# goodgodgd/xpt-mde-2021

Hardware: AMD Instinct MI355X
Metric: train images/sec (5-frame 128x416 snippets) (higher is better)
Workload: dtype bf16; 1 GPU; DepthNet(NASNetMobile)+PoseNetImproved train step, KITTI-raw-shaped 5x128x416 snippets, batch 8/GPU, mono L1+SSIM+smoothness, 4 scales; global_batch=8, per_gpu_batch=8, mode=graph, parallelism=dp1, ranks=1

## Files before the change

### include/xpt_hip.h

```cpp
#ifndef XPT_HIP_H_
#define XPT_HIP_H_

#include <stddef.h>
#include <stdint.h>

#ifdef __cplusplus
extern "C" {
#endif

#define XPT_OK 0
#define XPT_ERR_NULL (-1)
#define XPT_ERR_SHAPE (-2)
#define XPT_ERR_ARG (-3)
#define XPT_ERR_WORKSPACE (-4)
#define XPT_ERR_LAUNCH (-5)

#define XPT_PHOTO_L1 0
#define XPT_PHOTO_L2 1
#define XPT_PHOTO_SSIM 2

int xpt_abi_version(void);
const char* xpt_build_arch(void);

int xpt_pose_rvec2matr_fwd(const float* pose, float* T, int M, void* stream);
// ... 125 lines not shown
int xpt_pwconv_tune(int ksplit_min_cin, int ksplit_max_tiles);
int xpt_pwconv_bn_fwd(const void* x, const void* w, const float* gamma, const float* beta, const float* mean,
                      const float* var, float eps, const void* residual, void* ypre, void* y, long long M, int cin,
                      int cout, long long pitch_x, void* stream);

typedef struct xpt_conv_pack_job {
  const float* src;
  void* fwd;
  void* bwd;
  long long sn, sc, sh, sw;
  int N, T, KW, C, Cp, Np;
  long long first_block;
} xpt_conv_pack_job;
int xpt_conv_pack_job_bytes(void);
int xpt_conv_pack_weights(const void* jobs, int njobs, long long nblocks, void* stream);
int xpt_conv2d_tune(int plan);
int xpt_conv2d_fwd(const void* x, const void* w, const float* bias, void* y, int B, int PH, int PW, int C,
                   long long xpitch, int N, int KH, int KW, int stride, int pad_t, int pad_l, int OH, int OW,
                   long long ypitch, int upsample, float slope, void* stream);
int xpt_conv2d_bwd_data(const void* g, const void* wb, void* dx, int B, int OH, int OW, int Np, long long gpitch,
                        int C, int KH, int KW, int stride, int pad_t, int pad_l, int IH, int IW, long long dxpitch,
                        int fold2x2, void* stream);
int xpt_conv2d_splitk_tune(int enable, int force_split, int min_k, int max_pixels);
size_t xpt_conv2d_splitk_workspace_floats(long long pixels, int out_channels, int red_channels, int taps, int stride);
int xpt_conv2d_fwd_splitk(const void* x, const void* w, const float* bias, void* y, int B, int PH, int PW, int C,
                          long long xpitch, int N, int KH, int KW, int pad_t, int pad_l, int OH, int OW, long long ypitch,
                          int upsample, float slope, float* workspace, size_t workspace_floats, void* stream);
int xpt_conv2d_bwd_data_splitk(const void* g, const void* wb, void* dx, int B, int OH, int OW, int Np, long long gpitch,
                               int C, int KH, int KW, int pad_t, int pad_l, int IH, int IW, long long dxpitch, int fold2x2,
                               float* workspace, size_t workspace_floats, void* stream);
int xpt_conv2d_stream_tune(int enable, int min_tiles, int wgs_per_cu, int max_lds_kib);
int xpt_conv2d_stream_serves(int B, int OH, int OW, int out_channels, int red_channels, int KH, int KW, int stride,
                             int upsample_or_fold);
int xpt_conv2d_fwd_stream(const void* x, const void* w, const float* bias, void* y, int B, int PH, int PW, int C,
                          long long xpitch, int N, int pad_t, int pad_l, int OH, int OW, long long ypitch, int upsample,
                          float slope, void* stream);
int xpt_conv2d_fwd_stream_k5s2(const void* x, const void* w, const float* bias, void* y, int B, int PH, int PW, int C,
                               long long xpitch, int N, int pad_t, int pad_l, int OH, int OW, long long ypitch, float slope,
                               void* stream);
int xpt_conv2d_bwd_data_stream(const void* g, const void* wb, void* dx, int B, int OH, int OW, int Np, long long gpitch, int C,
                               int pad_t, int pad_l, int IH, int IW, long long dxpitch, int fold2x2, void* stream);
int xpt_conv2d_bwd_weight_tune(int max_partial_mib, int target_blocks);
int xpt_conv2d_bwd_weight_splits(int B, int C, int N, int KH, int KW, int stride, int OH, int OW);
int xpt_conv2d_bwd_weight_partials(const void* g, const void* x, float* partials, size_t partial_floats, int B, int PH,
                                   int PW, int C, int Cr, long long xpitch, int N, long long gpitch, int KH, int KW,
                                   int stride, int pad_t, int pad_l, int OH, int OW, int upsample, void* stream);
int xpt_restack_bf16(const float* image5d, void* out, int B, int S, int H, int W, int Cp, void* stream);

int xpt_headconv_tune(int passes, int max_blocks);
int xpt_headconv_bwd_blocks(int B, int H, int W, int C);
int xpt_headconv_fwd(const void* x, long long xpitch, const float* w, const float* bias, float* pre, int B, int H, int W,
                     int C, void* stream);
int xpt_headconv_bwd(const void* x, long long xpitch, const float* w, const float* g, void* dx, float* partials,
// ... 173 lines not shown
```

### xpt_mde_2021_amd/csrc/xpt_conv_splitk.hip

```cpp
#include "xpt_common.h"

namespace {

typedef float f32x16 __attribute__((ext_vector_type(16)));
typedef xpt_h16x8 bf16x8;
typedef unsigned int u32x4 __attribute__((ext_vector_type(4)));

__device__ inline unsigned short f2bf_sk(float f) { return xpt_f2h(f); }

struct SkArgs {
  const unsigned short* x;
  const unsigned short* w;
  float* part;
  long long xpitch;
  long long xbytes, wbytes;
  long long M;
  int B, PH, PW;
  int Hlim, Wlim, shift;
  int C, N, KH, KW;
  int sgn, off_h, off_w;
  int OH, OW, quad;
  int npieces, per_split, nsplit;
  int tiles_m, tiles_n;
};

template <int RN, int NW>
__global__ __launch_bounds__(64 * NW) void conv_splitk_kernel(SkArgs a) {
  constexpr int TN = 64 * RN, TP = 128, PITCH = 64 * 2 + 16;
  constexpr int RPP = 8 * NW, APASS = TN / RPP, BPASS = TP / RPP;
  constexpr int WI = NW == 4 ? RN : 1;
  static_assert(NW == 4 || (NW == 8 && RN == 2), "8 waves: the 128-channel tile only");
  __shared__ __attribute__((aligned(16))) unsigned char lds[(TN + TP) * PITCH];
  unsigned char* const lA = lds;
  unsigned char* const lB = lds + TN * PITCH;
  const int tid = threadIdx.x, lane = tid & 63, wave = tid >> 6;
  const int r = lane & 31, h = lane >> 5;
  const int wm = NW == 4 ? wave >> 1 : wave >> 2, wn = NW == 4 ? wave & 1 : wave & 3;

  const unsigned bid = blockIdx.x;
  int split, tile;
  if (a.nsplit >= 8) {
    split = (int)(bid % (unsigned)a.nsplit);
    tile = (int)(bid / (unsigned)a.nsplit);
  } else {
    const int per = 8 / a.nsplit;
    split = (int)(bid & 7u) % a.nsplit;
    tile = (int)(bid >> 3) * per + (int)(bid & 7u) / a.nsplit;
  }
  if (tile >= a.tiles_m * a.tiles_n) return;
  const int tn = tile % a.tiles_n, tm = tile / a.tiles_n;
  const long long m0 = (long long)tm * TP;
// ... 27 lines not shown

  const int sp = tid & 7, srow = tid >> 3;
  int sb[BPASS], base_h[BPASS], base_w[BPASS];
  bool sok[BPASS];
#pragma unroll
  for (int i = 0; i < BPASS; ++i) {
    int b, oh, ow;
    sok[i] = decode(m0 + srow + RPP * i, b, oh, ow);
    sb[i] = b;
    base_h[i] = oh + a.off_h;
    base_w[i] = ow + a.off_w;
  }
  const int T = a.KH * a.KW;
  constexpr unsigned OOB = 0x40000000u;
  unsigned wro[APASS];
#pragma unroll
  for (int i = 0; i < APASS; ++i) {
    const int n = n0 + srow + RPP * i;
    wro[i] = n < a.N ? (unsigned)n * (unsigned)(T * a.C) * 2u : OOB;
  }
  const __amdgpu_buffer_rsrc_t rx = __builtin_amdgcn_make_buffer_rsrc((void*)a.x, 0, (int)a.xbytes, 0x00020000);
  const __amdgpu_buffer_rsrc_t rw = __builtin_amdgcn_make_buffer_rsrc((void*)a.w, 0, (int)a.wbytes, 0x00020000);

  f32x16 acc[WI][2];
#pragma unroll
  for (int i = 0; i < WI; ++i)
#pragma unroll
    for (int j = 0; j < 2; ++j)
#pragma unroll
      for (int q = 0; q < 16; ++q) acc[i][j][q] = 0.f;

  int pc = p_begin + sp;
  int it, c0;
  {
    const int pcl = pc < a.npieces ? pc : a.npieces - 1;
    it = (int)(((float)pcl + 0.5f) * inv_cp8);
    c0 = (pcl - it * cp8) * 8;
  }
  unsigned xo[BPASS];
  auto set_tap = [&]() {
    const int kh = (int)(((float)it + 0.5f) * inv_kw);
    const int kw = it - kh * a.KW;
#pragma unroll
    for (int i = 0; i < BPASS; ++i) {
      const int th = base_h[i] + a.sgn * kh, tw = base_w[i] + a.sgn * kw;
      const bool ok = sok[i] && th >= 0 && th < a.Hlim && tw >= 0 && tw < a.Wlim;
      const int row = th >> a.shift, col = tw >> a.shift;
      xo[i] = ok ? (unsigned)((sb[i] * a.PH + row) * a.PW + col) * (unsigned)(a.xpitch * 2) : OOB;
    }
  };
  set_tap();
// ... 5 lines not shown
    const unsigned dead = pc < p_end ? 0u : OOB;
    const unsigned cb = (unsigned)(it * a.C + c0) * 2u + dead, xb = (unsigned)c0 * 2u + dead;
#pragma unroll
    for (int i = 0; i < APASS; ++i) st.ra[i] = __builtin_amdgcn_raw_buffer_load_b128(rw, wro[i] + cb, 0, 0);
#pragma unroll
    for (int i = 0; i < BPASS; ++i) st.rb[i] = __builtin_amdgcn_raw_buffer_load_b128(rx, xo[i] + xb, 0, 0);
    pc += 8;
    c0 += 64;
    if (c0 >= a.C) {
      do {
        c0 -= a.C;
        ++it;
      } while (c0 >= a.C);
      it = it < T ? it : T - 1;
      set_tap();
    }
  };
  auto stash = [&](const Stage& st) {
#pragma unroll
    for (int i = 0; i < APASS; ++i) *(u32x4*)(lA + (srow + RPP * i) * PITCH + sp * 16) = st.ra[i];
#pragma unroll
    for (int i = 0; i < BPASS; ++i) *(u32x4*)(lB + (srow + RPP * i) * PITCH + sp * 16) = st.rb[i];
  };
  const unsigned char* const fB = lB + (wm * 64 + r) * PITCH + h * 16;
  const unsigned char* const fA = lA + (wn * 32 * WI + r) * PITCH + h * 16;
  auto multiply = [&]() {
    u32x4 fb[4][2], fa[4][WI];
#pragma unroll
    for (int k16 = 0; k16 < 4; ++k16) {
#pragma unroll
      for (int j = 0; j < 2; ++j) fb[k16][j] = *(const u32x4*)(fB + 32 * j * PITCH + k16 * 32);
#pragma unroll
      for (int i = 0; i < WI; ++i) fa[k16][i] = *(const u32x4*)(fA + 32 * i * PITCH + k16 * 32);
    }
#pragma unroll
    for (int k16 = 0; k16 < 4; ++k16)
#pragma unroll
      for (int i = 0; i < WI; ++i)
#pragma unroll
        for (int j = 0; j < 2; ++j)
          acc[i][j] = XPT_MFMA_32X32X16(__builtin_bit_cast(bf16x8, fa[k16][i]), __builtin_bit_cast(bf16x8, fb[k16][j]),
                                                              acc[i][j]);
  };

  Stage s0, s1;
  if (nchunks > 0) {
    fetch(s0);
    if (nchunks > 1) fetch(s1);
    stash(s0);
    if (nchunks > 2) fetch(s0);
    __syncthreads();
  }
  for (int ck = 0; ck < nchunks; ck += 2) {
    multiply();
    if (ck + 1 < nchunks) {
      __syncthreads();
      stash(s1);
      if (ck + 3 < nchunks) fetch(s1);
      __syncthreads();
      multiply();
      if (ck + 2 < nchunks) {
        __syncthreads();
        stash(s0);
        if (ck + 4 < nchunks) fetch(s0);
        __syncthreads();
      }
    }
  }

  float* const out = a.part + (long long)split * a.M * a.N;
  const bool vec_ok = (a.N & 3) == 0;
#pragma unroll
  for (int j = 0; j < 2; ++j) {
    const long long m = m0 + 64 * wm + 32 * j + r;
    if (m >= a.M) continue;
#pragma unroll
    for (int i = 0; i < WI; ++i) {
#pragma unroll
      for (int qg = 0; qg < 4; ++qg) {
        const int n = n0 + 32 * WI * wn + 32 * i + 8 * qg + 4 * h;
        if (n >= a.N) continue;
        float* dst = out + m * a.N + n;
        if (vec_ok) {
          *(float4*)dst = make_float4(acc[i][j][4 * qg], acc[i][j][4 * qg + 1], acc[i][j][4 * qg + 2], acc[i][j][4 * qg + 3]);
        } else {
#pragma unroll
          for (int e = 0; e < 4; ++e)
            if (n + e < a.N) dst[e] = acc[i][j][4 * qg + e];
        }
      }
    }
  }
}

template <int NS>
__global__ __launch_bounds__(256) void conv_splitk_finish_kernel(const float* __restrict__ part, const float* __restrict__ bias,
                                                                 unsigned short* __restrict__ y, long long ypitch, unsigned Mout,
                                                                 long long M, int N, int quad, float slope) {
  const unsigned n4 = (unsigned)(N + 3) >> 2;
  const unsigned idx = blockIdx.x * 256u + threadIdx.x;
  if (idx >= Mout * n4) return;
  unsigned rem;
  const unsigned mo = xpt_divmod(idx, n4, rem);
  const int n = (int)rem * 4;
  const int nchild = quad ? 4 : 1;
  float s[4] = {0.f, 0.f, 0.f, 0.f};
  const bool vec = (N & 3) == 0;
  const long long slab = M * N;
  for (int c = 0; c < nchild; ++c) {
    const float* src = part + ((long long)mo * nchild + c) * N + n;
    if (vec) {
      float4 v[NS];
#pragma unroll
      for (int sp = 0; sp < NS; ++sp) v[sp] = *(const float4*)(src + sp * slab);
#pragma unroll
      for (int sp = 0; sp < NS; ++sp) { s[0] += v[sp].x; s[1] += v[sp].y; s[2] += v[sp].z; s[3] += v[sp].w; }
    } else {
#pragma unroll
      for (int sp = 0; sp < NS; ++sp)
#pragma unroll
        for (int e = 0; e < 4; ++e)
          if (n + e < N) s[e] += src[sp * slab + e];
    }
  }
#pragma unroll
  for (int e = 0; e < 4; ++e) {
    if (bias != nullptr && n + e < N) s[e] += bias[n + e];
    s[e] = s[e] > 0.f ? s[e] : s[e] * slope;
  }
  unsigned short* dst = y + (long long)mo * ypitch + n;
  if (vec && (ypitch & 3) == 0 && (((uintptr_t)y) & 7) == 0) {
    uint2 pk;
    pk.x = (unsigned)f2bf_sk(s[0]) | ((unsigned)f2bf_sk(s[1]) << 16);
    pk.y = (unsigned)f2bf_sk(s[2]) | ((unsigned)f2bf_sk(s[3]) << 16);
    *(uint2*)dst = pk;
  } else {
#pragma unroll
    for (int e = 0; e < 4; ++e)
      if (n + e < N) dst[e] = f2bf_sk(s[e]);
  }
}

int g_sk_skip_finish = 0;
int g_sk_waves = 8;
int g_sk_enable = 1;
int g_sk_force_split = 0;
int g_sk_min_k = 1024;
int g_sk_max_pixels = 8192;

struct SkPlan {
  int nsplit, per_split, tiles_m, tiles_n, rn;
};

SkPlan sk_plan(long long M, int N, int C, int T) {
  SkPlan p{};
  if (!g_sk_enable || (C & 7) != 0 || M <= 0 || M >= 0x7fffffffLL) return p;
  const long long K = (long long)C * T;
  if (!g_sk_force_split && (K < g_sk_min_k || M > g_sk_max_pixels || (M > 2048 && K < 1536))) return p;
  p.rn = N > 64 ? 2 : 1;
  const int TN = 64 * p.rn;
  p.tiles_m = (int)((M + 127) / 128);
  p.tiles_n = (N + TN - 1) / TN;
  const int tiles = p.tiles_m * p.tiles_n;
  const int npieces = (int)(K / 8);
  int ns = 1;
  if (g_sk_force_split > 0) {
    ns = g_sk_force_split;
  } else {
    while (ns < 16 && tiles * ns * 2 <= 320) ns *= 2;
    while (ns > 1 && npieces / ns < 32) ns >>= 1;
  }
  if (ns != 1 && ns != 2 && ns != 4 && ns != 8 && ns != 16) return SkPlan{};
  p.per_split = ((npieces + ns - 1) / ns + 7) & ~7;
  p.nsplit = ns;
  while (p.nsplit > 1 && (p.nsplit - 1) * p.per_split >= npieces) --p.nsplit;
  if (p.nsplit != 1 && p.nsplit != 2 && p.nsplit != 4 && p.nsplit != 8 && p.nsplit != 16) {
    int q = 1;
    while (q * 2 <= p.nsplit) q *= 2;
    p.nsplit = q;
    p.per_split = ((npieces + q - 1) / q + 7) & ~7;
  }
  return p;
}

int launch_sk(SkArgs& a, const SkPlan& p, const float* bias, unsigned short* y, long long ypitch, float slope, hipStream_t s) {
  a.nsplit = p.nsplit; a.per_split = p.per_split; a.tiles_m = p.tiles_m; a.tiles_n = p.tiles_n;
  const long long tiles = (long long)p.tiles_m * p.tiles_n;
  long long blocks;
  if (p.nsplit >= 8) blocks = tiles * p.nsplit;
  else {
    const int per = 8 / p.nsplit;
    blocks = ((tiles + per - 1) / per) * 8;
  }
  if (blocks > 0x7fffffffLL) return XPT_ERR_SHAPE;
  XPT_BEGIN_LAUNCH();
  if (p.rn == 2 && g_sk_waves == 8) hipLaunchKernelGGL((conv_splitk_kernel<2, 8>), dim3((unsigned)blocks), dim3(512), 0, s, a);
  else if (p.rn == 2) hipLaunchKernelGGL((conv_splitk_kernel<2, 4>), dim3((unsigned)blocks), dim3(256), 0, s, a);
  else hipLaunchKernelGGL((conv_splitk_kernel<1, 4>), dim3((unsigned)blocks), dim3(256), 0, s, a);
  const long long Mout = a.quad ? a.M / 4 : a.M;
  const long long threads = Mout * ((a.N + 3) / 4);
  if (g_sk_skip_finish) return xpt_launch_status();
  const dim3 fgrid((unsigned)((threads + 255) / 256));
#define SK_FINISH(NS) hipLaunchKernelGGL(conv_splitk_finish_kernel<NS>, fgrid, dim3(256), 0, s, a.part, bias, y, ypitch, (unsigned)Mout, \
                                         a.M, a.N, a.quad, slope)
  switch (p.nsplit) {
    case 1: SK_FINISH(1); break;
    case 2: SK_FINISH(2); break;
    case 4: SK_FINISH(4); break;
    case 8: SK_FINISH(8); break;
    default: SK_FINISH(16); break;
  }
#undef SK_FINISH
  return xpt_launch_status();
}

}

extern "C" int xpt_conv2d_splitk_tune(int enable, int force_split, int min_k, int max_pixels) {
  if (force_split < 0 || force_split > 16 || min_k < 0 || max_pixels < 0) return XPT_ERR_ARG;
  g_sk_enable = enable != 0;
  g_sk_skip_finish = enable == 2;
  if (enable >= 4) { g_sk_waves = enable; g_sk_enable = 1; }
  g_sk_force_split = force_split;
  if (min_k > 0) g_sk_min_k = min_k;
  if (max_pixels > 0) g_sk_max_pixels = max_pixels;
  return XPT_OK;
}

extern "C" size_t xpt_conv2d_splitk_workspace_floats(long long pixels, int out_channels, int red_channels, int taps, int stride) {
  if (stride != 1) return 0;
  const SkPlan p = sk_plan(pixels, out_channels, red_channels, taps);
  return p.nsplit ? (size_t)p.nsplit * (size_t)pixels * (size_t)out_channels : 0;
}

extern "C" int xpt_conv2d_fwd_splitk(const void* x, const void* w, const float* bias, void* y, int B, int PH, int PW, int C,
                                     long long xpitch, int N, int KH, int KW, int pad_t, int pad_l, int OH, int OW,
                                     long long ypitch, int upsample, float slope, float* workspace, size_t workspace_floats,
                                     void* stream) {
  XPT_CHECK_PTR(x); XPT_CHECK_PTR(w); XPT_CHECK_PTR(y); XPT_CHECK_PTR(workspace);
  if (B <= 0 || PH <= 0 || PW <= 0 || C <= 0 || N <= 0 || KH <= 0 || KW <= 0 || OH <= 0 || OW <= 0) return XPT_ERR_SHAPE;
  if (C % 8 != 0 || xpitch < C || xpitch % 8 != 0 || ypitch < N || ((uintptr_t)x) % 16 != 0 || ((uintptr_t)w) % 16 != 0 ||
      ((uintptr_t)workspace) % 16 != 0)
    return XPT_ERR_ARG;
  if ((upsample != 0 && upsample != 1) || pad_t < 0 || pad_l < 0) return XPT_ERR_ARG;
  SkArgs a{};
  a.x = (const unsigned short*)x; a.w = (const unsigned short*)w; a.part = workspace;
  a.xpitch = xpitch;
  a.B = B; a.PH = PH; a.PW = PW; a.shift = upsample; a.Hlim = PH << upsample; a.Wlim = PW << upsample;
  a.C = C; a.N = N; a.KH = KH; a.KW = KW;
  a.sgn = 1; a.off_h = -pad_t; a.off_w = -pad_l;
  a.OH = OH; a.OW = OW; a.quad = 0;
  a.M = (long long)B * OH * OW;
  a.npieces = KH * KW * (C / 8);
  if ((long long)(OH - 1) - pad_t >= a.Hlim || (long long)(OW - 1) - pad_l >= a.Wlim) return XPT_ERR_SHAPE;
  a.xbytes = ((long long)B * PH * PW - 1) * xpitch * 2 + (long long)C * 2;
  a.wbytes = (long long)N * KH * KW * C * 2;
  if (a.xbytes >= (1LL << 30) || a.wbytes >= (1LL << 30)) return XPT_ERR_SHAPE;
  const SkPlan p = sk_plan(a.M, N, C, KH * KW);
  if (!p.nsplit) return XPT_ERR_ARG;
  if (workspace_floats < (size_t)p.nsplit * (size_t)a.M * (size_t)N) return XPT_ERR_WORKSPACE;
  return launch_sk(a, p, bias, (unsigned short*)y, ypitch, slope, (hipStream_t)stream);
}

extern "C" int xpt_conv2d_bwd_data_splitk(const void* g, const void* wb, void* dx, int B, int OH, int OW, int Np, long long gpitch,
                                          int C, int KH, int KW, int pad_t, int pad_l, int IH, int IW, long long dxpitch,
                                          int fold2x2, float* workspace, size_t workspace_floats, void* stream) {
  XPT_CHECK_PTR(g); XPT_CHECK_PTR(wb); XPT_CHECK_PTR(dx); XPT_CHECK_PTR(workspace);
  if (B <= 0 || OH <= 0 || OW <= 0 || Np <= 0 || C <= 0 || KH <= 0 || KW <= 0 || IH <= 0 || IW <= 0) return XPT_ERR_SHAPE;
  if (Np % 8 != 0 || gpitch < Np || gpitch % 8 != 0 || dxpitch < C || ((uintptr_t)g) % 16 != 0 || ((uintptr_t)wb) % 16 != 0 ||
      ((uintptr_t)workspace) % 16 != 0)
    return XPT_ERR_ARG;
  if (fold2x2 != 0 && fold2x2 != 1) return XPT_ERR_ARG;
  SkArgs a{};
  a.x = (const unsigned short*)g; a.w = (const unsigned short*)wb; a.part = workspace;
  a.xpitch = gpitch;
  a.B = B; a.PH = OH; a.PW = OW; a.shift = 0; a.Hlim = OH; a.Wlim = OW;
  a.C = Np; a.N = C; a.KH = KH; a.KW = KW;
  a.sgn = -1; a.off_h = pad_t; a.off_w = pad_l;
  a.OH = fold2x2 ? 2 * IH : IH; a.OW = fold2x2 ? 2 * IW : IW; a.quad = fold2x2;
  if (fold2x2 && (a.OH != OH || a.OW != OW)) return XPT_ERR_SHAPE;
  a.M = (long long)B * a.OH * a.OW;
  a.npieces = KH * KW * (Np / 8);
  a.xbytes = ((long long)B * OH * OW - 1) * gpitch * 2 + (long long)Np * 2;
  a.wbytes = (long long)C * KH * KW * Np * 2;
  if (a.xbytes >= (1LL << 30) || a.wbytes >= (1LL << 30)) return XPT_ERR_SHAPE;
  const SkPlan p = sk_plan(a.M, C, Np, KH * KW);
  if (!p.nsplit) return XPT_ERR_ARG;
  if (workspace_floats < (size_t)p.nsplit * (size_t)a.M * (size_t)C) return XPT_ERR_WORKSPACE;
  return launch_sk(a, p, nullptr, (unsigned short*)dx, dxpitch, 1.f, (hipStream_t)stream);
}
```

### xpt_mde_2021_amd/hip/conv.py

```python
import contextlib
import ctypes
import math
import weakref

import torch

from . import lib as _lib
from . import ops as _ops


def _stream():
    return torch.cuda.current_stream().cuda_stream


def round_up(n, m):
    return (n + m - 1) // m * m


def same_pad(n, k, s):
    total = max((math.ceil(n / s) - 1) * s + k - n, 0)
    return total // 2, total - total // 2


class ConvWeightPacker:
# ... 7 lines not shown

    def get(self, weight, need_bwd=True):
        e = self.entries.get(id(weight))
        if e is not None and e["ref"]() is weight:
            if need_bwd and e["bwd"] is None:
                if torch.cuda.is_current_stream_capturing():
                    raise _lib.XptHipError("ConvWeightPacker: new operand layout requested during graph capture")
                e["bwd"] = torch.zeros((e["Cp"], e["T"], e["Np"]), dtype=_lib.half(), device=weight.device)
                self.signature = None
                self._pack_now()
            return e
        if torch.cuda.is_current_stream_capturing():
            raise _lib.XptHipError("ConvWeightPacker: a convolution weight was first used during graph capture "
                                   "(run one eager step first)")
        N, C, KH, KW = weight.shape
        Cp, Np, T = round_up(C, 8), round_up(N, 8), KH * KW
        e = {"ref": weakref.ref(weight), "N": N, "C": C, "KH": KH, "KW": KW, "T": T, "Cp": Cp, "Np": Np,
             "fwd": torch.zeros((N, T, Cp), dtype=_lib.half(), device=weight.device),
             "bwd": torch.zeros((Cp, T, Np), dtype=_lib.half(), device=weight.device) if need_bwd else None}
        self.entries[id(weight)] = e
        self.signature = None
        self._pack_now()
        return e

    def _live(self):
        dead = [k for k, e in self.entries.items() if e["ref"]() is None]
        for k in dead:
            del self.entries[k]
        if dead:
            self.signature = None
        return [(e["ref"](), e) for e in self.entries.values()]

    def _pack_now(self):
        if not torch.cuda.is_current_stream_capturing():
            self.pack()

    def pack(self):
        live = self._live()
        live = [(w, e) for w, e in live if w is not None and w.is_cuda]
        if not live:
            return
        lib = _lib.load()
        sig = tuple((w.data_ptr(), w.stride(), e["fwd"].data_ptr(), 0 if e["bwd"] is None else e["bwd"].data_ptr())
                    for w, e in live)
        if sig != self.signature:
            if torch.cuda.is_current_stream_capturing():
# ... 87 lines not shown
            _apply_env_tuning()
            _tuned = True
        x, xpitch = nhwc_view(x)
        B, Cx, PH, PW = x.shape
        need_dx = ctx.needs_input_grad[0]
        e = packer.get(weight, need_bwd=need_dx)
        N, C, KH, KW, Cp = e["N"], e["C"], e["KH"], e["KW"], e["Cp"]
        if Cx != Cp:
            raise _lib.XptHipError(f"conv: input has {Cx} channels, the packed weight expects {Cp} (= {C} padded to 8)")
        H, W = PH << upsample, PW << upsample
        if valid:
            pt = pl = 0
            OH, OW = (H - KH) // stride + 1, (W - KW) // stride + 1
        else:
            (pt, _), (pl, _) = same_pad(H, KH, stride), same_pad(W, KW, stride)
            OH, OW = -(-H // stride), -(-W // stride)
        y = torch.empty((B, N, OH, OW), dtype=_lib.half(), device=x.device, memory_format=torch.channels_last)
        b_ = None if bias is None else bias.detach()
        if b_ is not None and (b_.dtype != torch.float32 or not b_.is_contiguous()):
            raise _lib.XptHipError("conv: bias must be a contiguous float32 vector")
        wsf = 0 if valid else lib.xpt_conv2d_splitk_workspace_floats(B * OH * OW, N, Cp, KH * KW, stride)
        if wsf:
            ws = torch.empty(wsf, dtype=torch.float32, device=x.device)
            _lib.check(lib.xpt_conv2d_fwd_splitk(x.data_ptr(), e["fwd"].data_ptr(), None if b_ is None else b_.data_ptr(),
                                                 y.data_ptr(), B, PH, PW, Cp, xpitch, N, KH, KW, pt, pl, OH, OW, N,
                                                 int(upsample), float(slope), ws.data_ptr(), wsf, _stream()),
                       "xpt_conv2d_fwd_splitk")
        elif not valid and KH == 5 and lib.xpt_conv2d_stream_serves(B, OH, OW, N, Cp, KH, KW, stride, int(upsample)):
            _lib.check(lib.xpt_conv2d_fwd_stream_k5s2(x.data_ptr(), e["fwd"].data_ptr(), None if b_ is None else b_.data_ptr(),
                                                      y.data_ptr(), B, PH, PW, Cp, xpitch, N, pt, pl, OH, OW, N, float(slope),
                                                      _stream()), "xpt_conv2d_fwd_stream_k5s2")
        elif not valid and KH == 3 and lib.xpt_conv2d_stream_serves(B, OH, OW, N, Cp, KH, KW, stride, int(upsample)):
            _lib.check(lib.xpt_conv2d_fwd_stream(x.data_ptr(), e["fwd"].data_ptr(), None if b_ is None else b_.data_ptr(),
                                                 y.data_ptr(), B, PH, PW, Cp, xpitch, N, pt, pl, OH, OW, N, int(upsample),
                                                 float(slope), _stream()), "xpt_conv2d_fwd_stream")
        else:
            _lib.check(lib.xpt_conv2d_fwd(x.data_ptr(), e["fwd"].data_ptr(), None if b_ is None else b_.data_ptr(),
                                          y.data_ptr(), B, PH, PW, Cp, xpitch, N, KH, KW, stride, pt, pl, OH, OW, N,
                                          int(upsample), float(slope), _stream()), "xpt_conv2d_fwd")
        ctx.save_for_backward(x, y if slope != 1.0 else None, b_)
        ctx.geom = (B, PH, PW, Cp, C, xpitch, N, KH, KW, stride, pt, pl, OH, OW, int(upsample), float(slope))
        ctx.weight = weight
        ctx.sink_w = weight.flat_grad if (_ops.grad_sink.wants(weight) and N % 8 == 0) else None
        ctx.sink_b = bias.flat_grad if (bias is not None and _ops.grad_sink.wants(bias)) else None
        ctx.has_bias = bias is not None
        return y

    @staticmethod
    def backward(ctx, dy_in):
# ... 32 lines not shown
        dx = dw = None
        if ctx.needs_input_grad[1]:
            if ctx.sink_w is not None and WGRAD_DEFER and getattr(weight, "defer_wgrad", False):
                _deferred.append((ctx, g, gpitch, x))
                side = None
            else:
                side = _wgrad_side_stream(g.device) if (ctx.sink_w is not None and WGRAD_SIDE_STREAM) else None
            if _deferred and _deferred[-1][0] is ctx:
                pass
            elif side is not None:
                side.wait_stream(torch.cuda.current_stream())
                g.record_stream(side)
                x.record_stream(side)
                _ops.grad_sink.join_streams.add(side)
            if not (_deferred and _deferred[-1][0] is ctx):
                with torch.cuda.stream(side) if side is not None else contextlib.nullcontext():
                    dw = _weight_grad(ctx, lib, g, gpitch, x)
        if ctx.needs_input_grad[0]:
            e = packer.get(weight, need_bwd=True)
            dx = torch.empty((B, Cp, PH, PW), dtype=_lib.half(), device=g.device, memory_format=torch.channels_last)
            wsf = lib.xpt_conv2d_splitk_workspace_floats(B * (PH << ups) * (PW << ups), Cp, e["Np"], KH * KW, stride)
            if wsf:
                ws = torch.empty(wsf, dtype=torch.float32, device=g.device)
                _lib.check(lib.xpt_conv2d_bwd_data_splitk(g.data_ptr(), e["bwd"].data_ptr(), dx.data_ptr(), B, OH, OW, e["Np"],
                                                          gpitch, Cp, KH, KW, pt, pl, PH, PW, Cp, ups, ws.data_ptr(), wsf,
                                                          _stream()), "xpt_conv2d_bwd_data_splitk")
            elif KH == 3 and lib.xpt_conv2d_stream_serves(B, PH << ups, PW << ups, Cp, e["Np"], KH, KW, stride, ups):
                _lib.check(lib.xpt_conv2d_bwd_data_stream(g.data_ptr(), e["bwd"].data_ptr(), dx.data_ptr(), B, OH, OW, e["Np"],
                                                          gpitch, Cp, pt, pl, PH, PW, Cp, ups, _stream()),
                           "xpt_conv2d_bwd_data_stream")
            else:
                _lib.check(lib.xpt_conv2d_bwd_data(g.data_ptr(), e["bwd"].data_ptr(), dx.data_ptr(), B, OH, OW, e["Np"], gpitch,
                                                   Cp, KH, KW, stride, pt, pl, PH, PW, Cp, ups, _stream()), "xpt_conv2d_bwd_data")
        if _deferred and getattr(weight, "flush_wgrads", False):
            _flush_deferred(True)
        return dx, dw, dbias, None, None, None, None


WGRAD_DEFER = __import__("os").environ.get("XPT_WGRAD_DEFER", "0") == "1"
_deferred = []


def _flush_deferred(to_side):
    global _deferred
    queue, _deferred = _deferred, []
    if not queue:
        return
    lib = _lib.load()
    side = _wgrad_side_stream(queue[0][1].device) if to_side else None
# ... 188 lines not shown
```

### xpt_mde_2021_amd/hip/lib.py

```python
import ctypes
import os

_HERE = os.path.dirname(os.path.abspath(__file__))
LIB_PATH = os.environ.get("XPT_HIP_LIB") or os.path.join(os.path.dirname(_HERE), "libxpt_hip.so")
LIB_PATH_F16 = os.environ.get("XPT_HIP_LIB_F16") or os.path.join(os.path.dirname(_HERE), "libxpt_hip_f16.so")

_half_format = os.environ.get("XPT_HALF", "bf16")


def set_half_format(fmt):
    global _half_format
    if fmt not in ("bf16", "fp16"):
        raise XptHipError(f"unknown 16-bit format {fmt!r} (bf16 | fp16)")
    if _lib is not None and fmt != _half_format:
        raise XptHipError(f"the {_half_format} build of the library is already loaded in this process: {fmt} needs its own process "
                          f"(XPT_HALF={fmt} in the environment, or set_half_format() before the first op)")
    _half_format = fmt


def half_format():
    return _half_format


_half_dtype = None
# ... 128 lines not shown
    "xpt_pose_metric": (_i, [_p, _p, _p, _i, _i, _p]),
    "xpt_depth_metric": (_i, [_p, _p, _p, _i, _i, _i, _i, _i, _i, _i, _f, _f, _p]),
    "xpt_adjust_gather": (_i, [_p, ctypes.c_longlong, _p, _i, _i, _i, _i, _i, _p]),
    "xpt_adjust_scatter": (_i, [_p, ctypes.c_longlong, _p, ctypes.c_longlong, _p, _i, _i, _i, _i, _i, _p]),
    "xpt_pool_pair_fwd": (_i, [_p, ctypes.c_longlong, _p, _p, _p, _i, _i, _i, _i, _i, _i, _i, _i, _i, _p]),
    "xpt_pool_pair_bwd": (_i, [_p, ctypes.c_longlong, _p, ctypes.c_longlong, _p, _p, _i, _i, _i, _i, _i, _i, _i, _i, _i, _p]),
    "xpt_pool_pair_bwd2": (_i, [_p, ctypes.c_longlong, _p, ctypes.c_longlong, _p, ctypes.c_longlong, _p, _p, _i, _i, _i, _i, _i, _i,
                                _i, _i, _i, _p]),
    "xpt_cell_tail_fwd": (_i, [_i, _p, _p, _p, _p, _p, _p, ctypes.c_longlong, _i, _i, _i, _i, _i, _p]),
    "xpt_cell_tail_bwd": (_i, [_i, _p, _p, _p, ctypes.c_longlong, _p, _i, _i, _p, _p, _p, _p, _p, _i, _i, _i, _i, _i, _p]),
    "xpt_crc32c": (ctypes.c_uint32, [_p, _z]),
    "xpt_tfrecord_index": (ctypes.c_longlong, [_p, _z, _i, _p, _p, _p, ctypes.c_longlong]),
    "xpt_tfrecord_decode": (_i, [_p, _z, ctypes.c_uint32, _i, _i, _p, _p, _p]),
    "xpt_conv_pack_job_bytes": (_i, []),
    "xpt_conv_pack_weights": (_i, [_p, _i, ctypes.c_longlong, _p]),
    "xpt_conv2d_tune": (_i, [_i]),
    "xpt_conv2d_fwd": (_i, [_p, _p, _p, _p, _i, _i, _i, _i, ctypes.c_longlong, _i, _i, _i, _i, _i, _i, _i, _i,
                            ctypes.c_longlong, _i, _f, _p]),
    "xpt_conv2d_bwd_data": (_i, [_p, _p, _p, _i, _i, _i, _i, ctypes.c_longlong, _i, _i, _i, _i, _i, _i, _i, _i,
                                 ctypes.c_longlong, _i, _p]),
    "xpt_conv2d_splitk_tune": (_i, [_i, _i, _i, _i]),
    "xpt_conv2d_splitk_workspace_floats": (_z, [ctypes.c_longlong, _i, _i, _i, _i]),
    "xpt_conv2d_fwd_splitk": (_i, [_p, _p, _p, _p, _i, _i, _i, _i, ctypes.c_longlong, _i, _i, _i, _i, _i, _i, _i,
                                   ctypes.c_longlong, _i, _f, _p, _z, _p]),
    "xpt_conv2d_bwd_data_splitk": (_i, [_p, _p, _p, _i, _i, _i, _i, ctypes.c_longlong, _i, _i, _i, _i, _i, _i, _i,
                                        ctypes.c_longlong, _i, _p, _z, _p]),
    "xpt_conv2d_stream_tune": (_i, [_i, _i, _i, _i]),
    "xpt_conv2d_stream_serves": (_i, [_i] * 9),
    "xpt_conv2d_fwd_stream": (_i, [_p, _p, _p, _p, _i, _i, _i, _i, ctypes.c_longlong, _i, _i, _i, _i, _i, ctypes.c_longlong,
                                   _i, _f, _p]),
    "xpt_conv2d_fwd_stream_k5s2": (_i, [_p, _p, _p, _p, _i, _i, _i, _i, ctypes.c_longlong, _i, _i, _i, _i, _i, ctypes.c_longlong,
                                        _f, _p]),
    "xpt_conv2d_bwd_data_stream": (_i, [_p, _p, _p, _i, _i, _i, _i, ctypes.c_longlong, _i, _i, _i, _i, _i, ctypes.c_longlong,
                                        _i, _p]),
    "xpt_conv2d_bwd_weight_tune": (_i, [_i, _i]),
    "xpt_conv2d_bwd_weight_splits": (_i, [_i] * 8),
    "xpt_conv2d_bwd_weight_partials": (_i, [_p, _p, _p, _z, _i, _i, _i, _i, _i, ctypes.c_longlong, _i, ctypes.c_longlong,
                                            _i, _i, _i, _i, _i, _i, _i, _i, _p]),
    "xpt_headconv_bwd_blocks": (_i, [_i, _i, _i, _i]),
    "xpt_headconv_fwd": (_i, [_p, ctypes.c_longlong, _p, _p, _p, _i, _i, _i, _i, _p]),
    "xpt_headconv_bwd": (_i, [_p, ctypes.c_longlong, _p, _p, _p, _p, _z, _i, _i, _i, _i, _p]),
    "xpt_headconv_bwd_add": (_i, [_p, ctypes.c_longlong, _p, _p, _p, ctypes.c_longlong, _p, _p, _z, _i, _i, _i, _i, _p]),
    "xpt_restack_bf16": (_i, [_p, _p, _i, _i, _i, _i, _i, _p]),
    "xpt_affine_act_fwd": (_i, [_p, _p, _p, _p, _p, _f, _p, _p, ctypes.c_longlong, _i, _f, _i, _i, _p]),
    "xpt_affine_act_bwd_workspace_floats": (_z, [ctypes.c_longlong, _i]),
    "xpt_affine_act_bwd": (_i, [_p, _p, _p, ctypes.c_longlong, _p, _p, _p, _p, _f, _p, _p, _p, _p, _z, ctypes.c_longlong,
                                _i, _f, _i, _i, _p]),
}

# ... 52 lines not shown
```

Baseline: 1965 images/sec.

## Fuse split-K reduction into conv kernel via per-tile atomic counters; add 64-pixel tiles

```diff
diff --git a/include/xpt_hip.h b/include/xpt_hip.h
--- a/include/xpt_hip.h
+++ b/include/xpt_hip.h
@@ -171,13 +171,15 @@
                         int C, int KH, int KW, int stride, int pad_t, int pad_l, int IH, int IW, long long dxpitch,
                         int fold2x2, void* stream);
 int xpt_conv2d_splitk_tune(int enable, int force_split, int min_k, int max_pixels);
+int xpt_conv2d_splitk_counters(long long pixels, int out_channels, int red_channels, int taps, int stride);
 size_t xpt_conv2d_splitk_workspace_floats(long long pixels, int out_channels, int red_channels, int taps, int stride);
 int xpt_conv2d_fwd_splitk(const void* x, const void* w, const float* bias, void* y, int B, int PH, int PW, int C,
                           long long xpitch, int N, int KH, int KW, int pad_t, int pad_l, int OH, int OW, long long ypitch,
-                          int upsample, float slope, float* workspace, size_t workspace_floats, void* stream);
+                          int upsample, float slope, float* workspace, size_t workspace_floats, unsigned* counters,
+                          int n_counters, void* stream);
 int xpt_conv2d_bwd_data_splitk(const void* g, const void* wb, void* dx, int B, int OH, int OW, int Np, long long gpitch,
                                int C, int KH, int KW, int pad_t, int pad_l, int IH, int IW, long long dxpitch, int fold2x2,
-                               float* workspace, size_t workspace_floats, void* stream);
+                               float* workspace, size_t workspace_floats, unsigned* counters, int n_counters, void* stream);
 int xpt_conv2d_stream_tune(int enable, int min_tiles, int wgs_per_cu, int max_lds_kib);
 int xpt_conv2d_stream_serves(int B, int OH, int OW, int out_channels, int red_channels, int KH, int KW, int stride,
                              int upsample_or_fold);
diff --git a/xpt_mde_2021_amd/csrc/xpt_conv_splitk.hip b/xpt_mde_2021_amd/csrc/xpt_conv_splitk.hip
--- a/xpt_mde_2021_amd/csrc/xpt_conv_splitk.hip
+++ b/xpt_mde_2021_amd/csrc/xpt_conv_splitk.hip
@@ -1,4 +1,6 @@
 #include "xpt_common.h"
+
+#include <type_traits>
 
 namespace {
 
@@ -22,11 +24,63 @@
   int OH, OW, quad;
   int npieces, per_split, nsplit;
   int tiles_m, tiles_n;
+  unsigned* counters;
+  const float* bias;
+  unsigned short* y;
+  long long ypitch;
+  long long partbytes;
+  float slope;
 };
 
-template <int RN, int NW>
+template <int NS, bool SC1>
+__device__ inline void sk_finish_item(const float* __restrict__ part, __amdgpu_buffer_rsrc_t rpart, const float* __restrict__ bias,
+                                      unsigned short* __restrict__ y, long long ypitch, long long M, int N, int quad, float slope,
+                                      unsigned mo, int n) {
+  const int nchild = quad ? 4 : 1;
+  float s[4] = {0.f, 0.f, 0.f, 0.f};
+  const bool vec = SC1 || (N & 3) == 0;
+  const long long slab = M * N;
+  for (int c = 0; c < nchild; ++c) {
+    const long long at = ((long long)mo * nchild + c) * N + n;
+    if (vec) {
+      float4 v[NS];
+#pragma unroll
+      for (int sp = 0; sp < NS; ++sp) {
+        if (SC1) v[sp] = __builtin_bit_cast(float4, __builtin_amdgcn_raw_buffer_load_b128(rpart, (unsigned)((at + sp * slab) * 4), 0, 16));
+        else v[sp] = *(const float4*)(part + at + sp * slab);
+      }
+#pragma unroll
+      for (int sp = 0; sp < NS; ++sp) { s[0] += v[sp].x; s[1] += v[sp].y; s[2] += v[sp].z; s[3] += v[sp].w; }
+    } else {
+#pragma unroll
+      for (int sp = 0; sp < NS; ++sp)
+#pragma unroll
+        for (int e = 0; e < 4; ++e)
+          if (n + e < N) s[e] += part[at + sp * slab + e];
+    }
+  }
+#pragma unroll
+  for (int e = 0; e < 4; ++e) {
+    if (bias != nullptr && n + e < N) s[e] += bias[n + e];
+    s[e] = s[e] > 0.f ? s[e] : s[e] * slope;
+  }
+  unsigned short* dst = y + (long long)mo * ypitch + n;
+  if (vec && (ypitch & 3) == 0 && (((uintptr_t)y) & 7) == 0) {
+    uint2 pk;
+    pk.x = (unsigned)f2bf_sk(s[0]) | ((unsigned)f2bf_sk(s[1]) << 16);
+    pk.y = (unsigned)f2bf_sk(s[2]) | ((unsigned)f2bf_sk(s[3]) << 16);
+    *(uint2*)dst = pk;
+  } else {
+#pragma unroll
+    for (int e = 0; e < 4; ++e)
+      if (n + e < N) dst[e] = f2bf_sk(s[e]);
+  }
+}
+
+template <int RN, int NW, int TP>
 __global__ __launch_bounds__(64 * NW) void conv_splitk_kernel(SkArgs a) {
-  constexpr int TN = 64 * RN, TP = 128, PITCH = 64 * 2 + 16;
+  constexpr int TN = 64 * RN, PITCH = 64 * 2 + 16, PJ = TP / 64;
+  static_assert(TP == 128 || TP == 64, "pixel tile");
   constexpr int RPP = 8 * NW, APASS = TN / RPP, BPASS = TP / RPP;
   constexpr int WI = NW == 4 ? RN : 1;
   static_assert(NW == 4 || (NW == 8 && RN == 2), "8 waves: the 128-channel tile only");
@@ -100,11 +154,11 @@
   const __amdgpu_buffer_rsrc_t rx = __builtin_amdgcn_make_buffer_rsrc((void*)a.x, 0, (int)a.xbytes, 0x00020000);
   const __amdgpu_buffer_rsrc_t rw = __builtin_amdgcn_make_buffer_rsrc((void*)a.w, 0, (int)a.wbytes, 0x00020000);
 
-  f32x16 acc[WI][2];
+  f32x16 acc[WI][PJ];
 #pragma unroll
   for (int i = 0; i < WI; ++i)
 #pragma unroll
-    for (int j = 0; j < 2; ++j)
+    for (int j = 0; j < PJ; ++j)
 #pragma unroll
       for (int q = 0; q < 16; ++q) acc[i][j][q] = 0.f;
 
@@ -156,14 +210,14 @@
 #pragma unroll
     for (int i = 0; i < BPASS; ++i) *(u32x4*)(lB + (srow + RPP * i) * PITCH + sp * 16) = st.rb[i];
   };
-  const unsigned char* const fB = lB + (wm * 64 + r) * PITCH + h * 16;
+  const unsigned char* const fB = lB + (wm * 32 * PJ + r) * PITCH + h * 16;
   const unsigned char* const fA = lA + (wn * 32 * WI + r) * PITCH + h * 16;
   auto multiply = [&]() {
-    u32x4 fb[4][2], fa[4][WI];
+    u32x4 fb[4][PJ], fa[4][WI];
 #pragma unroll
     for (int k16 = 0; k16 < 4; ++k16) {
 #pragma unroll
-      for (int j = 0; j < 2; ++j) fb[k16][j] = *(const u32x4*)(fB + 32 * j * PITCH + k16 * 32);
+      for (int j = 0; j < PJ; ++j) fb[k16][j] = *(const u32x4*)(fB + 32 * j * PITCH + k16 * 32);
 #pragma unroll
       for (int i = 0; i < WI; ++i) fa[k16][i] = *(const u32x4*)(fA + 32 * i * PITCH + k16 * 32);
     }
@@ -172,7 +226,7 @@
 #pragma unroll
       for (int i = 0; i < WI; ++i)
 #pragma unroll
-        for (int j = 0; j < 2; ++j)
+        for (int j = 0; j < PJ; ++j)
           acc[i][j] = XPT_MFMA_32X32X16(__builtin_bit_cast(bf16x8, fa[k16][i]), __builtin_bit_cast(bf16x8, fb[k16][j]),
                                                               acc[i][j]);
   };
@@ -202,11 +256,13 @@
     }
   }
 
+  const bool inl = a.counters != nullptr;
   float* const out = a.part + (long long)split * a.M * a.N;
+  const __amdgpu_buffer_rsrc_t rpart = __builtin_amdgcn_make_buffer_rsrc((void*)a.part, 0, inl ? (int)a.partbytes : 0, 0x00020000);
   const bool vec_ok = (a.N & 3) == 0;
 #pragma unroll
-  for (int j = 0; j < 2; ++j) {
-    const long long m = m0 + 64 * wm + 32 * j + r;
+  for (int j = 0; j < PJ; ++j) {
+    const long long m = m0 + 32 * PJ * wm + 32 * j + r;
     if (m >= a.M) continue;
 #pragma unroll
     for (int i = 0; i < WI; ++i) {
@@ -215,8 +271,11 @@
         const int n = n0 + 32 * WI * wn + 32 * i + 8 * qg + 4 * h;
         if (n >= a.N) continue;
         float* dst = out + m * a.N + n;
-        if (vec_ok) {
-          *(float4*)dst = make_float4(acc[i][j][4 * qg], acc[i][j][4 * qg + 1], acc[i][j][4 * qg + 2], acc[i][j][4 * qg + 3]);
+        const float4 v4 = make_float4(acc[i][j][4 * qg], acc[i][j][4 * qg + 1], acc[i][j][4 * qg + 2], acc[i][j][4 * qg + 3]);
+        if (inl) {
+          __builtin_amdgcn_raw_buffer_store_b128(__builtin_bit_cast(u32x4, v4), rpart, (unsigned)((dst - a.part) * 4), 0, 16);
+        } else if (vec_ok) {
+          *(float4*)dst = v4;
         } else {
 #pragma unroll
           for (int e = 0; e < 4; ++e)
@@ -225,6 +284,43 @@
       }
     }
   }
+  if (!inl) return;
+
+  asm volatile("s_waitcnt vmcnt(0)" ::: "memory");
+  __syncthreads();
+  volatile unsigned* const last_flag = (volatile unsigned*)lds;
+  if (tid == 0) {
+    const unsigned arrived = __hip_atomic_fetch_add(a.counters + tile, 1u, __ATOMIC_RELAXED, __HIP_MEMORY_SCOPE_AGENT);
+    const unsigned last = arrived == (unsigned)a.nsplit - 1u ? 1u : 0u;
+    if (last) {
+      __builtin_amdgcn_fence(__ATOMIC_ACQUIRE, "agent");
+      asm volatile("s_waitcnt vmcnt(0)" ::: "memory");
+    }
+    *last_flag = last;
+  }
+  __syncthreads();
+  if (*last_flag == 0u) return;
+
+  constexpr int N4T = TN / 4;
+  const int rows_out = a.quad ? TP / 4 : TP;
+  const unsigned mo0 = (unsigned)(a.quad ? m0 >> 2 : m0), Mout = (unsigned)(a.quad ? a.M >> 2 : a.M);
+  auto finish = [&](auto ns_tag) {
+    constexpr int NS = decltype(ns_tag)::value;
+    for (int item = tid; item < rows_out * N4T; item += 64 * NW) {
+      const unsigned mo = mo0 + (unsigned)(item / N4T);
+      const int n = n0 + (item % N4T) * 4;
+      if (mo >= Mout || n >= a.N) continue;
+      sk_finish_item<NS, true>(a.part, rpart, a.bias, a.y, a.ypitch, a.M, a.N, a.quad, a.slope, mo, n);
+    }
+  };
+  switch (a.nsplit) {
+    case 1: finish(std::integral_constant<int, 1>{}); break;
+    case 2: finish(std::integral_constant<int, 2>{}); break;
+    case 4: finish(std::integral_constant<int, 4>{}); break;
+    case 8: finish(std::integral_constant<int, 8>{}); break;
+    default: finish(std::integral_constant<int, 16>{}); break;
+  }
+  if (tid == 0) __hip_atomic_store(a.counters + tile, 0u, __ATOMIC_RELAXED, __HIP_MEMORY_SCOPE_AGENT);
 }
 
 template <int NS>
@@ -236,46 +332,13 @@
   if (idx >= Mout * n4) return;
   unsigned rem;
   const unsigned mo = xpt_divmod(idx, n4, rem);
-  const int n = (int)rem * 4;
-  const int nchild = quad ? 4 : 1;
-  float s[4] = {0.f, 0.f, 0.f, 0.f};
-  const bool vec = (N & 3) == 0;
-  const long long slab = M * N;
-  for (int c = 0; c < nchild; ++c) {
-    const float* src = part + ((long long)mo * nchild + c) * N + n;
-    if (vec) {
-      float4 v[NS];
-#pragma unroll
-      for (int sp = 0; sp < NS; ++sp) v[sp] = *(const float4*)(src + sp * slab);
-#pragma unroll
-      for (int sp = 0; sp < NS; ++sp) { s[0] += v[sp].x; s[1] += v[sp].y; s[2] += v[sp].z; s[3] += v[sp].w; }
-    } else {
-#pragma unroll
-      for (int sp = 0; sp < NS; ++sp)
-#pragma unroll
-        for (int e = 0; e < 4; ++e)
-          if (n + e < N) s[e] += src[sp * slab + e];
-    }
-  }
-#pragma unroll
-  for (int e = 0; e < 4; ++e) {
-    if (bias != nullptr && n + e < N) s[e] += bias[n + e];
-    s[e] = s[e] > 0.f ? s[e] : s[e] * slope;
-  }
-  unsigned short* dst = y + (long long)mo * ypitch + n;
-  if (vec && (ypitch & 3) == 0 && (((uintptr_t)y) & 7) == 0) {
-    uint2 pk;
-    pk.x = (unsigned)f2bf_sk(s[0]) | ((unsigned)f2bf_sk(s[1]) << 16);
-    pk.y = (unsigned)f2bf_sk(s[2]) | ((unsigned)f2bf_sk(s[3]) << 16);
-    *(uint2*)dst = pk;
-  } else {
-#pragma unroll
-    for (int e = 0; e < 4; ++e)
-      if (n + e < N) dst[e] = f2bf_sk(s[e]);
-  }
+  const __amdgpu_buffer_rsrc_t none = __builtin_amdgcn_make_buffer_rsrc((void*)part, 0, 0, 0x00020000);
+  sk_finish_item<NS, false>(part, none, bias, y, ypitch, M, N, quad, slope, mo, (int)rem * 4);
 }
 
 int g_sk_skip_finish = 0;
+int g_sk_two_launch = 0;
+int g_sk_tile = 0;
 int g_sk_waves = 8;
 int g_sk_enable = 1;
 int g_sk_force_split = 0;
@@ -283,7 +346,7 @@
 int g_sk_max_pixels = 8192;
 
 struct SkPlan {
-  int nsplit, per_split, tiles_m, tiles_n, rn;
+  int nsplit, per_split, tiles_m, tiles_n, rn, tp;
 };
 
 SkPlan sk_plan(long long M, int N, int C, int T) {
@@ -293,6 +356,7 @@
   if (!g_sk_force_split && (K < g_sk_min_k || M > g_sk_max_pixels || (M > 2048 && K < 1536))) return p;
   p.rn = N > 64 ? 2 : 1;
   const int TN = 64 * p.rn;
+  p.tp = 128;
   p.tiles_m = (int)((M + 127) / 128);
   p.tiles_n = (N + TN - 1) / TN;
   const int tiles = p.tiles_m * p.tiles_n;
@@ -314,10 +378,15 @@
     p.nsplit = q;
     p.per_split = ((npieces + q - 1) / q + 7) & ~7;
   }
+  if (g_sk_tile == 64 || (g_sk_tile == 0 && (long long)tiles * p.nsplit < 512 && M > 64)) {
+    p.tp = 64;
+    p.tiles_m = (int)((M + 63) / 64);
+  }
   return p;
 }
 
-int launch_sk(SkArgs& a, const SkPlan& p, const float* bias, unsigned short* y, long long ypitch, float slope, hipStream_t s) {
+int launch_sk(SkArgs& a, const SkPlan& p, const float* bias, unsigned short* y, long long ypitch, float slope, unsigned* counters,
+              int n_counters, hipStream_t s) {
   a.nsplit = p.nsplit; a.per_split = p.per_split; a.tiles_m = p.tiles_m; a.tiles_n = p.tiles_n;
   const long long tiles = (long long)p.tiles_m * p.tiles_n;
   long long blocks;
@@ -327,13 +396,24 @@
     blocks = ((tiles + per - 1) / per) * 8;
   }
   if (blocks > 0x7fffffffLL) return XPT_ERR_SHAPE;
+  a.partbytes = (long long)p.nsplit * a.M * a.N * 4;
+  const bool inl = counters != nullptr && !g_sk_two_launch && !g_sk_skip_finish && (a.N & 3) == 0 && a.partbytes < (1LL << 31);
+  if (inl && n_counters < tiles) return XPT_ERR_WORKSPACE;
+  a.counters = inl ? counters : nullptr;
+  a.bias = bias; a.y = y; a.ypitch = ypitch; a.slope = slope;
   XPT_BEGIN_LAUNCH();
-  if (p.rn == 2 && g_sk_waves == 8) hipLaunchKernelGGL((conv_splitk_kernel<2, 8>), dim3((unsigned)blocks), dim3(512), 0, s, a);
-  else if (p.rn == 2) hipLaunchKernelGGL((conv_splitk_kernel<2, 4>), dim3((unsigned)blocks), dim3(256), 0, s, a);
-  else hipLaunchKernelGGL((conv_splitk_kernel<1, 4>), dim3((unsigned)blocks), dim3(256), 0, s, a);
+#define SK_TILES(TP)                                                                                                              \
+  do {                                                                                                                            \
+    if (p.rn == 2 && g_sk_waves == 8) hipLaunchKernelGGL((conv_splitk_kernel<2, 8, TP>), dim3((unsigned)blocks), dim3(512), 0, s, a); \
+    else if (p.rn == 2) hipLaunchKernelGGL((conv_splitk_kernel<2, 4, TP>), dim3((unsigned)blocks), dim3(256), 0, s, a);            \
+    else hipLaunchKernelGGL((conv_splitk_kernel<1, 4, TP>), dim3((unsigned)blocks), dim3(256), 0, s, a);                           \
+  } while (0)
+  if (p.tp == 64) SK_TILES(64);
+  else SK_TILES(128);
+#undef SK_TILES
   const long long Mout = a.quad ? a.M / 4 : a.M;
   const long long threads = Mout * ((a.N + 3) / 4);
-  if (g_sk_skip_finish) return xpt_launch_status();
+  if (g_sk_skip_finish || inl) return xpt_launch_status();
   const dim3 fgrid((unsigned)((threads + 255) / 256));
 #define SK_FINISH(NS) hipLaunchKernelGGL(conv_splitk_finish_kernel<NS>, fgrid, dim3(256), 0, s, a.part, bias, y, ypitch, (unsigned)Mout, \
                                          a.M, a.N, a.quad, slope)
@@ -354,7 +434,10 @@
   if (force_split < 0 || force_split > 16 || min_k < 0 || max_pixels < 0) return XPT_ERR_ARG;
   g_sk_enable = enable != 0;
   g_sk_skip_finish = enable == 2;
-  if (enable >= 4) { g_sk_waves = enable; g_sk_enable = 1; }
+  g_sk_two_launch = enable == 3;
+  if (enable == 4 || enable == 8) g_sk_waves = enable;
+  if (enable == 64 || enable == 128) g_sk_tile = enable;
+  if (enable == 192) g_sk_tile = 0;
   g_sk_force_split = force_split;
   if (min_k > 0) g_sk_min_k = min_k;
   if (max_pixels > 0) g_sk_max_pixels = max_pixels;
@@ -367,10 +450,17 @@
   return p.nsplit ? (size_t)p.nsplit * (size_t)pixels * (size_t)out_channels : 0;
 }
 
+extern "C" int xpt_conv2d_splitk_counters(long long pixels, int out_channels, int red_channels, int taps, int stride) {
+  if (stride != 1) return 0;
+  const SkPlan p = sk_plan(pixels, out_channels, red_channels, taps);
+  const long long tiles = p.nsplit ? ((pixels + 63) / 64) * p.tiles_n : 0;
+  return tiles > 0x7fffffffLL ? 0 : (int)tiles;
+}
+
 extern "C" int xpt_conv2d_fwd_splitk(const void* x, const void* w, const float* bias, void* y, int B, int PH, int PW, int C,
                                      long long xpitch, int N, int KH, int KW, int pad_t, int pad_l, int OH, int OW,
                                      long long ypitch, int upsample, float slope, float* workspace, size_t workspace_floats,
-                                     void* stream) {
+                                     unsigned* counters, int n_counters, void* stream) {
   XPT_CHECK_PTR(x); XPT_CHECK_PTR(w); XPT_CHECK_PTR(y); XPT_CHECK_PTR(workspace);
   if (B <= 0 || PH <= 0 || PW <= 0 || C <= 0 || N <= 0 || KH <= 0 || KW <= 0 || OH <= 0 || OW <= 0) return XPT_ERR_SHAPE;
   if (C % 8 != 0 || xpitch < C || xpitch % 8 != 0 || ypitch < N || ((uintptr_t)x) % 16 != 0 || ((uintptr_t)w) % 16 != 0 ||
@@ -393,12 +483,13 @@
   const SkPlan p = sk_plan(a.M, N, C, KH * KW);
   if (!p.nsplit) return XPT_ERR_ARG;
   if (workspace_floats < (size_t)p.nsplit * (size_t)a.M * (size_t)N) return XPT_ERR_WORKSPACE;
-  return launch_sk(a, p, bias, (unsigned short*)y, ypitch, slope, (hipStream_t)stream);
+  return launch_sk(a, p, bias, (unsigned short*)y, ypitch, slope, counters, n_counters, (hipStream_t)stream);
 }
 
 extern "C" int xpt_conv2d_bwd_data_splitk(const void* g, const void* wb, void* dx, int B, int OH, int OW, int Np, long long gpitch,
                                           int C, int KH, int KW, int pad_t, int pad_l, int IH, int IW, long long dxpitch,
-                                          int fold2x2, float* workspace, size_t workspace_floats, void* stream) {
+                                          int fold2x2, float* workspace, size_t workspace_floats, unsigned* counters,
+                                          int n_counters, void* stream) {
   XPT_CHECK_PTR(g); XPT_CHECK_PTR(wb); XPT_CHECK_PTR(dx); XPT_CHECK_PTR(workspace);
   if (B <= 0 || OH <= 0 || OW <= 0 || Np <= 0 || C <= 0 || KH <= 0 || KW <= 0 || IH <= 0 || IW <= 0) return XPT_ERR_SHAPE;
   if (Np % 8 != 0 || gpitch < Np || gpitch % 8 != 0 || dxpitch < C || ((uintptr_t)g) % 16 != 0 || ((uintptr_t)wb) % 16 != 0 ||
@@ -421,5 +512,5 @@
   const SkPlan p = sk_plan(a.M, C, Np, KH * KW);
   if (!p.nsplit) return XPT_ERR_ARG;
   if (workspace_floats < (size_t)p.nsplit * (size_t)a.M * (size_t)C) return XPT_ERR_WORKSPACE;
-  return launch_sk(a, p, nullptr, (unsigned short*)dx, dxpitch, 1.f, (hipStream_t)stream);
-}
+  return launch_sk(a, p, nullptr, (unsigned short*)dx, dxpitch, 1.f, counters, n_counters, (hipStream_t)stream);
+}
diff --git a/xpt_mde_2021_amd/hip/conv.py b/xpt_mde_2021_amd/hip/conv.py
--- a/xpt_mde_2021_amd/hip/conv.py
+++ b/xpt_mde_2021_amd/hip/conv.py
@@ -53,6 +53,15 @@
         self.signature = None
         self._pack_now()
         return e
+
+    def splitk_counters(self, e, direction, count):
+        t = e.get("sk_" + direction)
+        if t is None or t.numel() < count:
+            if torch.cuda.is_current_stream_capturing():
+                raise _lib.XptHipError("ConvWeightPacker: split-K tile counters first requested during graph capture "
+                                       "(run one eager step first)")
+            t = e["sk_" + direction] = torch.zeros(count, dtype=torch.int32, device=e["fwd"].device)
+        return t
 
     def _live(self):
         dead = [k for k, e in self.entries.items() if e["ref"]() is None]
@@ -186,9 +195,11 @@
         wsf = 0 if valid else lib.xpt_conv2d_splitk_workspace_floats(B * OH * OW, N, Cp, KH * KW, stride)
         if wsf:
             ws = torch.empty(wsf, dtype=torch.float32, device=x.device)
+            cnt = packer.splitk_counters(e, "fwd", lib.xpt_conv2d_splitk_counters(B * OH * OW, N, Cp, KH * KW, stride))
             _lib.check(lib.xpt_conv2d_fwd_splitk(x.data_ptr(), e["fwd"].data_ptr(), None if b_ is None else b_.data_ptr(),
                                                  y.data_ptr(), B, PH, PW, Cp, xpitch, N, KH, KW, pt, pl, OH, OW, N,
-                                                 int(upsample), float(slope), ws.data_ptr(), wsf, _stream()),
+                                                 int(upsample), float(slope), ws.data_ptr(), wsf, cnt.data_ptr(), cnt.numel(),
+                                                 _stream()),
                        "xpt_conv2d_fwd_splitk")
         elif not valid and KH == 5 and lib.xpt_conv2d_stream_serves(B, OH, OW, N, Cp, KH, KW, stride, int(upsample)):
             _lib.check(lib.xpt_conv2d_fwd_stream_k5s2(x.data_ptr(), e["fwd"].data_ptr(), None if b_ is None else b_.data_ptr(),
@@ -267,9 +278,11 @@
             wsf = lib.xpt_conv2d_splitk_workspace_floats(B * (PH << ups) * (PW << ups), Cp, e["Np"], KH * KW, stride)
             if wsf:
                 ws = torch.empty(wsf, dtype=torch.float32, device=g.device)
+                cnt = packer.splitk_counters(e, "bwd", lib.xpt_conv2d_splitk_counters(B * (PH << ups) * (PW << ups), Cp, e["Np"],
+                                                                                      KH * KW, stride))
                 _lib.check(lib.xpt_conv2d_bwd_data_splitk(g.data_ptr(), e["bwd"].data_ptr(), dx.data_ptr(), B, OH, OW, e["Np"],
                                                           gpitch, Cp, KH, KW, pt, pl, PH, PW, Cp, ups, ws.data_ptr(), wsf,
-                                                          _stream()), "xpt_conv2d_bwd_data_splitk")
+                                                          cnt.data_ptr(), cnt.numel(), _stream()), "xpt_conv2d_bwd_data_splitk")
             elif KH == 3 and lib.xpt_conv2d_stream_serves(B, PH << ups, PW << ups, Cp, e["Np"], KH, KW, stride, ups):
                 _lib.check(lib.xpt_conv2d_bwd_data_stream(g.data_ptr(), e["bwd"].data_ptr(), dx.data_ptr(), B, OH, OW, e["Np"],
                                                           gpitch, Cp, pt, pl, PH, PW, Cp, ups, _stream()),
diff --git a/xpt_mde_2021_amd/hip/lib.py b/xpt_mde_2021_amd/hip/lib.py
--- a/xpt_mde_2021_amd/hip/lib.py
+++ b/xpt_mde_2021_amd/hip/lib.py
@@ -174,9 +174,10 @@
     "xpt_conv2d_splitk_tune": (_i, [_i, _i, _i, _i]),
     "xpt_conv2d_splitk_workspace_floats": (_z, [ctypes.c_longlong, _i, _i, _i, _i]),
     "xpt_conv2d_fwd_splitk": (_i, [_p, _p, _p, _p, _i, _i, _i, _i, ctypes.c_longlong, _i, _i, _i, _i, _i, _i, _i,
-                                   ctypes.c_longlong, _i, _f, _p, _z, _p]),
+                                   ctypes.c_longlong, _i, _f, _p, _z, _p, _i, _p]),
     "xpt_conv2d_bwd_data_splitk": (_i, [_p, _p, _p, _i, _i, _i, _i, ctypes.c_longlong, _i, _i, _i, _i, _i, _i, _i,
-                                        ctypes.c_longlong, _i, _p, _z, _p]),
+                                        ctypes.c_longlong, _i, _p, _z, _p, _i, _p]),
+    "xpt_conv2d_splitk_counters": (_i, [ctypes.c_longlong, _i, _i, _i, _i]),
     "xpt_conv2d_stream_tune": (_i, [_i, _i, _i, _i]),
     "xpt_conv2d_stream_serves": (_i, [_i] * 9),
     "xpt_conv2d_fwd_stream": (_i, [_p, _p, _p, _p, _i, _i, _i, _i, ctypes.c_longlong, _i, _i, _i, _i, _i, ctypes.c_longlong,
```

Result: no change. 1967 images/sec, median of 2 (+0.1%).
